# LMCache/LMCache

Hardware: AMD Instinct MI355X
Metric: KV encode+offload GB/s per GPU -- value = CacheGen encode, HBM -> HBM (raw 16-bit KV bytes consumed, PCIe never inside value); the PCIe-inclusive encode+offload rate is offload.encode_plus_offload_GBps_raw_kv (higher is better)
Workload: dtype bf16->u8 symbols (fp32 quantise, u32 rANS); 1 GPU; Llama-3-8B bf16 KV, 16384-token context, CacheGen encode, chunk_size=256 (BASELINE configs[1]); layers=32, kv_heads=8, head_dim=128, chunks=64, raw_kv_bytes=2147483648, numa_node=0

## Files before the change

lmcache_amd/csrc/k_encode_counts.h:

```cpp
#pragma once
#include "k_encode.h"

#define RTAB_ENTRIES 257
#define RTAB_DWORDS (2 * RTAB_ENTRIES + 2)
struct RansRtab {
  u32 v[RTAB_DWORDS];
};
constexpr RansRtab make_rans_rtab() {
  RansRtab t{};
  for (u32 c = 1; c <= 256u; c++) {
    const u32 f = 2u * c;
    u32 l = 1;
    while ((1u << l) < f) l++;
    const u64 num = 1ull << (31u + l);
    t.v[2 * c] = (u32)((num + f - 1u) / f);
    t.v[2 * c + 1] = (512u - f) | ((l - 1u) << 24);
  }
  return t;
}
__device__ const RansRtab g_rans_rtab = make_rans_rtab();
#define BITS_DWORDS 132
#define RTAB_LDS_DWORDS (RTAB_DWORDS + 2 * BITS_DWORDS)
struct CountsBits {
  u32 v[2 * BITS_DWORDS];
};
constexpr CountsBits make_counts_bits() {
  constexpr u16 t[257] = {LMC_COUNTS_BITS_LIST};
  constexpr u16 o[257] = {LMC_COUNTS_BPO_LIST};
  CountsBits r{};
  for (int i = 0; i < 257; i++) r.v[i >> 1] |= (u32)t[i] << (16 * (i & 1));
  for (int i = 0; i < 257; i++) r.v[BITS_DWORDS + (i >> 1)] |= (u32)o[i] << (16 * (i & 1));
  return r;
}
__device__ const CountsBits g_counts_bits = make_counts_bits();
#define CNT_RING_DWORDS 128

__device__ __forceinline__ void rtab_to_lds(u32* rtab_lds) {
  for (u32 i = threadIdx.x; i < RTAB_DWORDS; i += blockDim.x) rtab_lds[i] = g_rans_rtab.v[i];
  for (u32 i = threadIdx.x; i < 2 * BITS_DWORDS; i += blockDim.x) rtab_lds[RTAB_DWORDS + i] = g_counts_bits.v[i];
}

#define LMC_SYM_LAST_LOAD(p) __builtin_nontemporal_load((const LMC_GLOBAL u32*)(p))

#define CNT_TAB_DWORDS 1024

template <int POS, int WIDTH, int SHIFT>
__device__ __forceinline__ u32 row_addr_sh(u32 w, u32 base) {
  constexpr u32 FIELD = ((1u << WIDTH) - 1u);
  u32 r;
  if constexpr (POS == SHIFT) {
    asm("v_and_b32_e32 %0, %2, %1\n\tv_add_u32_e32 %0, %0, %3" : "=&v"(r) : "v"(w), "s"(FIELD << SHIFT), "v"(base));
  } else if constexpr (POS + WIDTH == 32) {
    asm("v_lshrrev_b32_e32 %0, %2, %1\n\tv_lshl_add_u32 %0, %0, %3, %4"
        : "=&v"(r) : "v"(w), "n"(POS), "n"(SHIFT), "v"(base));
  } else {
    asm("v_bfe_u32 %0, %1, %2, %3\n\tv_lshl_add_u32 %0, %0, %4, %5"
        : "=&v"(r) : "v"(w), "n"(POS), "n"(WIDTH), "n"(SHIFT), "v"(base));
  }
  return r;
}
template <bool NIB, int I, bool ALIGNED = false>
__device__ __forceinline__ u32 row_addr_cnt(const u32* w, u32 base) {
  if constexpr (NIB) {
    constexpr int POS = 8 * (I & 3) + 4 * ((I >> 2) & 1);
    if constexpr (ALIGNED && POS == 8) {
      u32 r;
      asm("v_and_or_b32 %0, %1, %2, %3" : "=v"(r) : "v"(w[I >> 3]), "s"(0xf00u), "v"(base));
      return r;
    } else if constexpr (ALIGNED && POS > 8) {
      u32 r;
      asm("v_lshrrev_b32_e32 %0, %2, %1\n\tv_and_or_b32 %0, %0, %3, %4" : "=&v"(r) : "v"(w[I >> 3]), "n"(POS - 8), "s"(0xf00u), "v"(base));
      return r;
    } else {
      return row_addr_sh<POS, 4, 8>(w[I >> 3], base);
    }
  } else {
    constexpr int POS = 8 * (I & 3);
    if constexpr (ALIGNED && POS >= 8) {
      u32 r;
      asm("v_lshrrev_b32_e32 %0, %2, %1\n\tv_and_or_b32 %0, %0, %3, %4" : "=&v"(r) : "v"(w[I >> 2]), "n"(POS - 7), "s"(0xf80u), "v"(base));
      return r;
    } else {
      return row_addr_sh<POS, 8, 7>(w[I >> 2], base);
    }
  }
}


struct CountsStream {
  int chunk, p, g, c;
  int T;
  bool active, nib;
  const u32* symq;
  u32 R;
};
__device__ __forceinline__ CountsStream counts_stream_of(const EncodeArgs& a, int chunk, int p, int g, int lane) {
  CountsStream s;
  s.g = g;
  s.p = p;
  s.chunk = chunk;
  s.c = s.g * 64 + lane;
  s.T = min(a.chunk_tokens, a.tok_end - (a.tok_begin + chunk * a.chunk_tokens));
  s.active = s.c < a.C;
  s.symq = a.sym4 + ((long long)s.chunk * a.P + s.p) * a.sym_stride + s.c;
  s.nib = lmc_sym_nibbles((int)a.bins.b[s.p]);
  s.R = (u32)a.bins.b[s.p] - 1u;
  return s;
}

struct CountsState {
  u32 pk[8];
  u32 wor[8];
  u32 head;
};

#define LMC_SDWA_BYTE_OP(NAME, OP)                                                                                      \
  template <int K>                                                                                                      \
  __device__ __forceinline__ u32 NAME(u32 a, u32 b) {                                                                   \
    u32 d;                                                                                                              \
    if constexpr (K == 0) asm(OP " %0, %1, %2 dst_sel:DWORD dst_unused:UNUSED_PAD src0_sel:DWORD src1_sel:BYTE_0" : "=v"(d) : "v"(a), "v"(b)); \
    else if constexpr (K == 1) asm(OP " %0, %1, %2 dst_sel:DWORD dst_unused:UNUSED_PAD src0_sel:DWORD src1_sel:BYTE_1" : "=v"(d) : "v"(a), "v"(b)); \
    else if constexpr (K == 2) asm(OP " %0, %1, %2 dst_sel:DWORD dst_unused:UNUSED_PAD src0_sel:DWORD src1_sel:BYTE_2" : "=v"(d) : "v"(a), "v"(b)); \
    else asm(OP " %0, %1, %2 dst_sel:DWORD dst_unused:UNUSED_PAD src0_sel:DWORD src1_sel:BYTE_3" : "=v"(d) : "v"(a), "v"(b)); \
    return d;                                                                                                           \
  }
LMC_SDWA_BYTE_OP(sdwa_byte_shl, "v_lshlrev_b32_sdwa")
LMC_SDWA_BYTE_OP(sdwa_byte_add, "v_add_u32_sdwa")
LMC_SDWA_BYTE_OP(sdwa_byte_or, "v_or_b32_sdwa")

template <int NS>
__device__ __forceinline__ void counts_model_pk(const u32 (&pk)[8], bool active, u32 T, u32 (&mp)[NS / 4]) {
  if (T == LMC_COUNTS_T) {
    u32 sum = 0;
#pragma unroll
    for (int k = 0; k < NS / 4; k++) sum = __builtin_amdgcn_sad_u8(pk[k], 0u, sum);
    const u32 deficit = LMC_COUNTS_T - sum;
    const bool first = (pk[0] & 0xffu) == 255u;
#pragma unroll
    for (int k = 0; k < NS / 4; k++) mp[k] = pk[k];
    mp[0] += first ? deficit << 8 : deficit;
  } else {
    const u32 magic = lmc_counts_scale_magic_dev(T);
    u32 cum = 0, prev = 0, big = 0, first = 0;
#pragma unroll
    for (int k = 0; k < NS / 4; k++) mp[k] = 0;
    static_for<NS>([&](auto itag) {
      constexpr int i = decltype(itag)::value;
      cum += (pk[i >> 2] >> (8 * (i & 3))) & 0xffu;
      const u32 now = __umulhi(cum << 8, magic);
      u32 n = now - prev;
      prev = now;
      if (n >= LMC_COUNTS_T) { big = 1u; first = i == 0 ? 1u : 0u; n = LMC_COUNTS_T - 1u; }
      mp[i >> 2] |= n << (8 * (i & 3));
    });
    if (big) mp[0] += first ? 1u << 8 : 1u;
  }
  if (!active) mp[0] = 0x01ffu;
}
__device__ __forceinline__ void counts_table_nib_pk(const u32 (&mp)[4], u32* tabmem, int lane) {
  u32 acc = 0;
  static_for<16>([&](auto itag) {
    constexpr int i = decltype(itag)::value;
    const u32 t = sdwa_byte_shl<i & 3>(23u, mp[i >> 2]);
    tabmem[i * 64 + lane] = (acc << 1) | t;
    acc = sdwa_byte_add<i & 3>(acc, mp[i >> 2]);
  });
}
__device__ __forceinline__ void counts_table_byte_pk(const u32 (&mp)[8], u16* tab16, int lane) {
  u32 acc = 0;
  static_for<32>([&](auto itag) {
    constexpr int i = decltype(itag)::value;
    tab16[i * 64 + lane] = (u16)sdwa_byte_or<i & 3>(acc << 8, mp[i >> 2]);
    acc = sdwa_byte_add<i & 3>(acc, mp[i >> 2]);
  });
}

template <bool ALIGNED = false, bool PLANE = false>
__device__ __forceinline__ u32 counts_hist_stream(const EncodeArgs& a, const CountsStream& s, u32* tabmem,
                                                  const u32* bits,
                                                  int lane, CountsState& cs, u32 vq_base = 0) {
  typedef __attribute__((address_space(3))) u32* lds_u32w;
  typedef const __attribute__((address_space(3))) u16* lds_u16p;
  typedef const __attribute__((address_space(3))) u8* lds_u8p;
  const int Tc = __builtin_amdgcn_readfirstlane(s.T);
  const u32 tab_addr = (u32)(size_t)(lds_u32w)tabmem;
  if (ALIGNED && (tab_addr & 0xfffu)) __builtin_trap();
  u16* const tab16 = reinterpret_cast<u16*>(tabmem);
  auto pass1 = [&](auto nib_tag) {
    constexpr bool NIB = decltype(nib_tag)::value;
    constexpr int DPB = NIB ? 4 : 8;
    const int NB = Tc >> 5, rem = Tc & 31;
    const int rows = NIB ? (Tc + 7) >> 3 : (Tc + 3) >> 2;
#pragma unroll
    for (int i = 0; i < 16; i++) tabmem[i * 64 + lane] = 0;
    const u32 col = NIB ? tab_addr + 4u * (u32)lane : tab_addr + 4u * (u32)(lane >> 1);
    const u32 one = NIB ? 1u : 1u << ((lane & 1) * 16);
    u32 w[DPB], wn[DPB];
#pragma unroll
    for (int j = 0; j < DPB; j++) w[j] = (s.active && j < rows) ? s.symq[(long long)j * a.C] : 0u;
    for (int b = 0; b < NB; b++) {
      if (b + 1 < NB || rem) {
#pragma unroll
        for (int j = 0; j < DPB; j++)
          wn[j] = (s.active && (b + 1) * DPB + j < rows) ? s.symq[(long long)((b + 1) * DPB + j) * a.C] : 0u;
      }
      static_for<32>([&](auto itag) {
        constexpr int i = decltype(itag)::value;
        const u32 ad = row_addr_cnt<NIB, i, ALIGNED>(w, col);
        __hip_atomic_fetch_add((lds_u32w)(size_t)ad, one, __ATOMIC_RELAXED, __HIP_MEMORY_SCOPE_WAVEFRONT);
      });
#pragma unroll
      for (int j = 0; j < DPB; j++) w[j] = wn[j];
    }
    for (int i = 0; i < rem; i++) {
      const int j = NIB ? i >> 3 : i >> 2;
      u32 wd = w[0];
#pragma unroll
      for (int k = 1; k < DPB; k++) wd = j == k ? w[k] : wd;
      const u32 sym = NIB ? (wd >> (8 * (i & 3) + 4 * ((i >> 2) & 1))) & 15u : (wd >> (8 * (i & 3))) & 0xffu;
      const u32 ad = col + (sym << (NIB ? 8 : 7));
      __hip_atomic_fetch_add((lds_u32w)(size_t)ad, one, __ATOMIC_RELAXED, __HIP_MEMORY_SCOPE_WAVEFRONT);
    }
  };
  const u32 vq = vq_base + (((u32)s.g) << 3) + ((u32)lane >> 3);
  const u32 qx = vq & 63u, qe = (u32)lane & 7u, qit = vq >> 6;
  u32 ph = 0;
  if constexpr (PLANE) {
    if (s.nib) {
      ph = (qit * 4u + (qe >> 1)) * 4096u + 4u * qx + 2u * (qe & 1u);
    } else {
      ph = (qit * 2u + (qe >> 2)) * 8192u + 4u * qx + (qe & 3u);
      const u32 sym0 = s.active ? (s.symq[0] & 0xffu) : 0u;
      const u32 a0 = ph + (sym0 << 8);
      const u32 c0 = (u32) * (lds_u8p)(size_t)a0;
      if (s.active && c0 != 255u)
        __hip_atomic_fetch_add((lds_u32w)(size_t)(a0 & ~3u), 1u << (8u * (a0 & 3u)), __ATOMIC_RELAXED, __HIP_MEMORY_SCOPE_WORKGROUP);
    }
  } else {
    if (s.nib) pass1(BoolTag<true>{});
    else pass1(BoolTag<false>{});
  }
  wave_lds_fence();

  if (s.g == 0) {
    const BlobOff bo = lmc_blob_off((u32)a.P, (u32)Tc, (u32)a.G);
    u8* const blob0 = a.blobs + (long long)s.chunk * a.blob_stride;
    const u32 sum = scale_checksum(reinterpret_cast<const u16*>(blob0 + bo.scales) + (long long)s.p * Tc, (u32)Tc, lane);
    if (lane == 0) reinterpret_cast<u32*>(blob0 + bo.scsum)[s.p] = sum;
  }
#pragma unroll
  for (int k = 0; k < 8; k++) cs.pk[k] = 0u;
  const u32 cap = s.active ? 255u : 0u;
  auto put = [&](auto itag, u32 c) {
    constexpr int i = decltype(itag)::value;
    if constexpr ((i & 3) == 0)
      asm("v_min_u32_sdwa %0, %1, %2 dst_sel:BYTE_0 dst_unused:UNUSED_PRESERVE src0_sel:DWORD src1_sel:DWORD" : "+v"(cs.pk[i >> 2]) : "v"(c), "v"(cap));
    else if constexpr ((i & 3) == 1)
      asm("v_min_u32_sdwa %0, %1, %2 dst_sel:BYTE_1 dst_unused:UNUSED_PRESERVE src0_sel:DWORD src1_sel:DWORD" : "+v"(cs.pk[i >> 2]) : "v"(c), "v"(cap));
    else if constexpr ((i & 3) == 2)
      asm("v_min_u32_sdwa %0, %1, %2 dst_sel:BYTE_2 dst_unused:UNUSED_PRESERVE src0_sel:DWORD src1_sel:DWORD" : "+v"(cs.pk[i >> 2]) : "v"(c), "v"(cap));
    else
      asm("v_min_u32_sdwa %0, %1, %2 dst_sel:BYTE_3 dst_unused:UNUSED_PRESERVE src0_sel:DWORD src1_sel:DWORD" : "+v"(cs.pk[i >> 2]) : "v"(c), "v"(cap));
  };
  if constexpr (PLANE) {
    if (s.nib) static_for<16>([&](auto itag) { put(itag, (u32) * (lds_u16p)(size_t)(ph + 256u * decltype(itag)::value)); });
    else static_for<32>([&](auto itag) { put(itag, (u32) * (lds_u8p)(size_t)(ph + 256u * decltype(itag)::value)); });
  } else {
    if (s.nib) static_for<16>([&](auto itag) { put(itag, tabmem[decltype(itag)::value * 64 + lane]); });
    else static_for<32>([&](auto itag) { put(itag, (u32)tab16[decltype(itag)::value * 64 + lane]); });
  }
  wave_lds_fence();
  head_or_counts<8>(cs.pk, cs.wor);
  cs.head = head_bytes_of<8, 8>(cs.wor, s.R);
  __builtin_assume(bits != nullptr);
  const u32 bits_addr = (u32)(size_t)(lds_u16p) reinterpret_cast<const u16*>(bits);
  u32 S = 0;
  auto bound = [&](auto ns_tag) {
    constexpr int NS = decltype(ns_tag)::value;
    u32 sum = 0;
#pragma unroll
    for (int k = 0; k < NS / 4; k++) sum = __builtin_amdgcn_sad_u8(cs.pk[k], 0u, sum);
    static_for<NS>([&](auto itag) {
      constexpr int i = decltype(itag)::value;
      u32 c2;
      if constexpr ((i & 3) == 0) asm("v_lshlrev_b32_sdwa %0, 1, %1 dst_sel:DWORD dst_unused:UNUSED_PAD src0_sel:DWORD src1_sel:BYTE_0" : "=v"(c2) : "v"(cs.pk[i >> 2]));
      else if constexpr ((i & 3) == 1) asm("v_lshlrev_b32_sdwa %0, 1, %1 dst_sel:DWORD dst_unused:UNUSED_PAD src0_sel:DWORD src1_sel:BYTE_1" : "=v"(c2) : "v"(cs.pk[i >> 2]));
      else if constexpr ((i & 3) == 2) asm("v_lshlrev_b32_sdwa %0, 1, %1 dst_sel:DWORD dst_unused:UNUSED_PAD src0_sel:DWORD src1_sel:BYTE_2" : "=v"(c2) : "v"(cs.pk[i >> 2]));
      else asm("v_lshlrev_b32_sdwa %0, 1, %1 dst_sel:DWORD dst_unused:UNUSED_PAD src0_sel:DWORD src1_sel:BYTE_3" : "=v"(c2) : "v"(cs.pk[i >> 2]));
      S += (u32) * (lds_u16p)(size_t)(c2 + bits_addr);
    });
    const u32 bits_of_1 = (u32) * (lds_u16p)(size_t)(bits_addr + 2u);
    S += sum == LMC_COUNTS_T - 1u ? bits_of_1 : 0u;
  };
  auto bound_T = [&](auto ns_tag) {
    constexpr int NS = decltype(ns_tag)::value;
    const u32 magic = lmc_counts_scale_magic_dev((u32)Tc);
    const u32 bpo_addr = bits_addr + 4u * BITS_DWORDS;
    u32 cum = 0, prev = 0;
    static_for<NS>([&](auto itag) {
      constexpr int i = decltype(itag)::value;
      const u32 c = (cs.pk[i >> 2] >> (8 * (i & 3))) & 0xffu;
      cum += c;
      const u32 now = __umulhi(cum << 8, magic);
      const u32 n = min(now - prev, LMC_COUNTS_T - 1u);
      prev = now;
      S += c * (u32) * (lds_u16p)(size_t)(bpo_addr + 2u * n);
    });
  };
  if (Tc == (int)LMC_COUNTS_T) {
    if (s.nib) bound(IntTag<16>{});
    else bound(IntTag<32>{});
  } else {
    if (s.nib) bound_T(IntTag<16>{});
    else bound_T(IntTag<32>{});
  }
  const u32 lw = s.active ? (S + 6u * ((S >> 12) + 2u)) >> 12 : 0u;
  const u32 words = (u32)__builtin_amdgcn_readfirstlane((int)wave_sum_u32(lw));
  return (cs.head + 2u * (words + 128u) + 15u) & ~15u;
}

__device__ __forceinline__ void counts_open_stream(const CountsStream& s, const CountsState& cs, u8* out, u32* tabmem, int lane) {
  (void)head_write<8, 8>(out, cs.pk, cs.wor, s.R, tabmem, lane);
  wave_lds_fence();
  if (s.nib) {
    u32 mp[4];
    counts_model_pk<16>(cs.pk, s.active, (u32)s.T, mp);
    counts_table_nib_pk(mp, tabmem, lane);
  } else {
    u32 mp[8];
    counts_model_pk<32>(cs.pk, s.active, (u32)s.T, mp);
    counts_table_byte_pk(mp, reinterpret_cast<u16*>(tabmem), lane);
  }
  wave_lds_fence();
}

template <bool NT>
__device__ __forceinline__ u32 counts_code_stream(const EncodeArgs& a, const CountsStream& s, u32* tabmem, u16* const ring,
                                                  const u32* rtab, int lane, u16* const out_v) {
  typedef __attribute__((address_space(3))) u32* lds_u32w;
  typedef __attribute__((address_space(3))) u16* lds_u16w;
  const int Tc = __builtin_amdgcn_readfirstlane(s.T);
  const u32 tab_addr = (u32)(size_t)(lds_u32w)tabmem;
  if (NT && (tab_addr & 0xfffu)) __builtin_trap();
  const u32 rtab_addr = (u32)__builtin_amdgcn_readfirstlane((int)(u32)(size_t)(lds_u32w) const_cast<u32*>(rtab));
  u32 x = s.active ? LMC_COUNTS_L : 0u;
  const u32 ring_addr = (u32)__builtin_amdgcn_readfirstlane((int)(u32)(size_t)(lds_u16w)ring);
  const u64 full_exec = __builtin_amdgcn_read_exec();
  u16* const out = reinterpret_cast<u16*>(uniform_ptr64(out_v));
  const u32 pre = (u32)__builtin_amdgcn_readfirstlane((int)((u32)(size_t)out & 255u));
  u32 skip = pre;
  u32 wb = ring_addr + pre;
  const u32 wlimit = ring_addr + 256u;
  u32 flushed = 0;
  const __amdgpu_buffer_rsrc_t out_rsrc = __builtin_amdgcn_make_buffer_rsrc((void*)((u8*)out - pre), (short)0, (int)0xfffffff0u, 0x00020000);
  auto flush_ring = [&]() {
    if (__builtin_expect(wb >= wlimit, 0)) {
      wave_lds_fence();
      u32 lane_here = (u32)lane;
      asm volatile("" : "+v"(lane_here));
      const u32 slot_addr = ring_addr + 4u * lane_here;
      const u32 v = *(lds_u32w)(size_t)slot_addr;
      const u32 up = *(lds_u32w)(size_t)(slot_addr + 256u);
      const u32 voff = 4u * lane_here;
#ifndef LMC_EXP_ENC_NO_FLUSH
      if (voff >= skip) __builtin_amdgcn_raw_buffer_store_b32((int)v, out_rsrc, (int)voff, (int)(flushed << 1), NT ? 2 : 0);
      skip = 0;
#else
      asm volatile("" :: "v"(v), "v"(voff));
#endif
      if (voff < wb - wlimit) *(lds_u32w)(size_t)slot_addr = up;
      flushed += 128u;
      wb -= 256u;
    }
  };
  auto rans_put_nib = [&](u32 e, u32 m, u32 shc) {
    u32 q;
    asm("v_mul_hi_u32 %[q], %[x], %[m]\n\t"
        "v_lshrrev_b32_sdwa %[q], %[shc], %[q] dst_sel:DWORD dst_unused:UNUSED_PAD src0_sel:BYTE_3 src1_sel:DWORD\n\t"
        "v_mad_u32_u24 %[x], %[q], %[shc], %[x]\n\t"
        "v_add_u32_sdwa %[x], %[x], %[e] dst_sel:DWORD dst_unused:UNUSED_PAD src0_sel:DWORD src1_sel:WORD_0"
        : [x] "+v"(x), [q] "=&v"(q)
        : [m] "v"(m), [shc] "v"(shc), [e] "v"(e));
  };
  auto rans_put_byte = [&](_Float16 e, u32 m, u32 shc) {
    u32 q, st2;
    asm("v_mul_hi_u32 %[q], %[x], %[m]\n\t"
        "v_lshrrev_b32_sdwa %[q], %[shc], %[q] dst_sel:DWORD dst_unused:UNUSED_PAD src0_sel:BYTE_3 src1_sel:DWORD\n\t"
        "v_lshlrev_b32_sdwa %[st2], 1, %[e] dst_sel:DWORD dst_unused:UNUSED_PAD src0_sel:DWORD src1_sel:BYTE_1\n\t"
        "v_mad_u32_u24 %[x], %[q], %[shc], %[x]\n\t"
        "v_add_u32_e32 %[x], %[x], %[st2]"
        : [x] "+v"(x), [q] "=&v"(q), [st2] "=&v"(st2)
        : [m] "v"(m), [shc] "v"(shc), [e] "v"(e));
  };

  auto pass2 = [&](auto nib_tag) {
    constexpr bool NIB = decltype(nib_tag)::value;
    constexpr int DPB = NIB ? 4 : 8;
    const int NB = Tc >> 5, rem = Tc & 31;
    const int rows = NIB ? (Tc + 7) >> 3 : (Tc + 3) >> 2;
    const u32 col = NIB ? tab_addr + 4u * (u32)lane : tab_addr + 2u * (u32)lane;
    using ET = std::conditional_t<NIB, u32, _Float16>;
    auto entry_at = [&](u32 ad) -> ET {
      if constexpr (NIB) return *(lds_u32w)(size_t)ad;
      else return __builtin_bit_cast(_Float16, *(lds_u16w)(size_t)ad);
    };
    auto rtab_of = [&](ET e) -> u32x2_t {
      u32 ra;
      if constexpr (NIB) ra = e >> 20;
      else ra = ((u32)__builtin_bit_cast(u16, e) & 0xffu) << 3;
      return *(const __attribute__((address_space(3))) u32x2_t*)(size_t)(rtab_addr + ra);
    };
    auto emit = [&](ET e0, ET e2, u32& ra) {
      u32 tt, cnt, wbn;
      if constexpr (NIB) {
        asm volatile("v_lshrrev_b32_e32 %[ra], 20, %[e2]\n\t"
                     "v_cmpx_ge_u32_sdwa vcc, %[x], %[e0] src0_sel:WORD_1 src1_sel:WORD_1\n\t"
                     "s_bcnt1_i32_b64 %[cnt], vcc\n\t"
                     "s_lshl1_add_u32 %[wbn], %[cnt], %[wb]\n\t"
                     "v_mbcnt_lo_u32_b32 %[t], vcc_lo, 0\n\t"
                     "v_mbcnt_hi_u32_b32 %[t], vcc_hi, %[t]\n\t"
                     "v_lshl_add_u32 %[t], %[t], 1, %[wb]\n\t"
                     "ds_write_b16 %[t], %[x]\n\t"
                     "v_lshrrev_b32_e32 %[x], 16, %[x]\n\t"
                     "s_mov_b64 exec, %[full]"
                     : [x] "+v"(x), [t] "=&v"(tt), [cnt] "=&s"(cnt), [wbn] "=&s"(wbn), [ra] "=&v"(ra)
                     : [e0] "v"(e0), [e2] "v"(e2), [wb] "s"(wb), [full] "s"(full_exec)
                     : "vcc", "scc", "memory");
      } else {
        asm volatile("v_lshlrev_b32_sdwa %[ra], 3, %[e2] dst_sel:DWORD dst_unused:UNUSED_PAD src0_sel:DWORD src1_sel:BYTE_0\n\t"
                     "v_lshlrev_b32_sdwa %[t], 23, %[e0] dst_sel:DWORD dst_unused:UNUSED_PAD src0_sel:DWORD src1_sel:BYTE_0\n\t"
                     "v_cmpx_ge_u32_e32 vcc, %[x], %[t]\n\t"
                     "s_bcnt1_i32_b64 %[cnt], vcc\n\t"
                     "s_lshl1_add_u32 %[wbn], %[cnt], %[wb]\n\t"
                     "v_mbcnt_lo_u32_b32 %[t], vcc_lo, 0\n\t"
                     "v_mbcnt_hi_u32_b32 %[t], vcc_hi, %[t]\n\t"
                     "v_lshl_add_u32 %[t], %[t], 1, %[wb]\n\t"
                     "ds_write_b16 %[t], %[x]\n\t"
                     "v_lshrrev_b32_e32 %[x], 16, %[x]\n\t"
                     "s_mov_b64 exec, %[full]"
                     : [x] "+v"(x), [t] "=&v"(tt), [cnt] "=&s"(cnt), [wbn] "=&s"(wbn), [ra] "=&v"(ra)
                     : [e0] "v"(e0), [e2] "v"(e2), [wb] "s"(wb), [full] "s"(full_exec)
                     : "vcc", "scc", "memory");
      }
      wb = wbn;
    };
    u32 w[DPB], wn[DPB];
#pragma unroll
    for (int j = 0; j < DPB; j++) {
      w[j] = (NB > 0 && s.active) ? LMC_SYM_LAST_LOAD(s.symq + (long long)((NB - 1) * DPB + j) * a.C) : 0u;
      wn[j] = (rem && s.active && NB * DPB + j < rows) ? LMC_SYM_LAST_LOAD(s.symq + (long long)(NB * DPB + j) * a.C) : 0u;
    }
    for (int i = rem - 1; i >= 0; i--) {
      const int j = NIB ? i >> 3 : i >> 2;
      u32 wd = wn[0];
#pragma unroll
      for (int k = 1; k < DPB; k++) wd = j == k ? wn[k] : wd;
      const u32 sym = NIB ? (wd >> (8 * (i & 3) + 4 * ((i >> 2) & 1))) & 15u : (wd >> (8 * (i & 3))) & 0xffu;
      const ET E = entry_at(col + (sym << (NIB ? 8 : 7)));
      const u32x2_t R = rtab_of(E);
      u32 ra_unused;
      emit(E, E, ra_unused);
      flush_ring();
      if constexpr (NIB) rans_put_nib(E, R.x, R.y);
      else rans_put_byte(E, R.x, R.y);
    }
#ifdef LMC_EXP_SKIP_TOKEN_LOOP
    return;
#endif
    if (NB == 0) return;
    ET E0 = entry_at(row_addr_cnt<NIB, 31, NT>(w, col));
    ET E1 = entry_at(row_addr_cnt<NIB, 30, NT>(w, col));
    ET E2 = entry_at(row_addr_cnt<NIB, 29, NT>(w, col));
    ET E3 = entry_at(row_addr_cnt<NIB, 28, NT>(w, col));
    u32x2_t R0 = rtab_of(E0);
    u32x2_t R1 = rtab_of(E1);
    for (int b = NB - 1; b >= 0; b--) {
#pragma unroll
      for (int j = 0; j < DPB; j++) wn[j] = (b > 0 && s.active) ? LMC_SYM_LAST_LOAD(s.symq + (long long)((b - 1) * DPB + j) * a.C) : 0u;
      static_for<32>([&](auto itag) {
        constexpr int i = 31 - decltype(itag)::value;
        u32 ad4;
        if constexpr (i >= 4) ad4 = row_addr_cnt<NIB, i - 4, NT>(w, col);
        else ad4 = row_addr_cnt<NIB, 28 + i, NT>(wn, col);
        u32 ra;
        emit(E0, E2, ra);
        const u32x2_t R2 = *(const __attribute__((address_space(3))) u32x2_t*)(size_t)(rtab_addr + ra);
        const ET E4 = entry_at(ad4);
        if constexpr ((i & 1) == 0) flush_ring();
        if constexpr (NIB) rans_put_nib(E0, R0.x, R0.y);
        else rans_put_byte(E0, R0.x, R0.y);
        E0 = E1; E1 = E2; E2 = E3; E3 = E4;
        R0 = R1; R1 = R2;
      });
#pragma unroll
      for (int j = 0; j < DPB; j++) w[j] = wn[j];
    }
  };
  if (s.nib) pass2(BoolTag<true>{});
  else pass2(BoolTag<false>{});
  x = s.active ? x : LMC_COUNTS_L;
  flush_ring();
  wave_lds_fence();
  const u32 pend_b = wb - ring_addr;
  {
    const u32 sa = wb + 4u * (u32)lane;
    *(lds_u16w)(size_t)sa = (u16)x;
    *(lds_u16w)(size_t)(sa + 2u) = (u16)(x >> 16);
  }
  wave_lds_fence();
  const u32 tot_b = pend_b + 256u;
  const u32 end_b = (tot_b + 15u) & ~15u;
  const u32 exact = (flushed << 1) + tot_b - pre;
#pragma unroll
  for (int h = 0; h < 2; h++) {
    const u32 voff = 256u * (u32)h + 4u * (u32)lane;
    if (voff < end_b && voff >= skip) {
      u32 v = *(lds_u32w)(size_t)(ring_addr + voff);
      v = voff >= tot_b ? 0u : (voff + 2u == tot_b ? (v & 0xffffu) : v);
      __builtin_amdgcn_raw_buffer_store_b32((int)v, out_rsrc, (int)voff, (int)(flushed << 1), NT ? 2 : 0);
    }
  }
  return exact;
}

template <bool QUADSYM, bool ENCODE, int NW = ENC_WAVES, bool COUNTS_ONLY = false>
__global__ __launch_bounds__(64 * NW) __attribute__((amdgpu_waves_per_eu(NW == 8 ? 8 : 4, 8))) void k_cdf_encode(EncodeArgs a) {
  static_assert(!COUNTS_ONLY || (QUADSYM && ENCODE), "the counts coder reads the workspace and places its streams");
  constexpr int TAB_DWORDS = COUNTS_ONLY ? CNT_TAB_DWORDS : ENC_TAB_DWORDS;
  constexpr int RING_DWORDS = COUNTS_ONLY ? CNT_RING_DWORDS : ENC_RING_DWORDS;
  __shared__ __attribute__((aligned(4096))) u32 lds_all[NW * (TAB_DWORDS + RING_DWORDS)];
  __shared__ __attribute__((aligned(16))) u32 rtab_lds[ENCODE ? RTAB_LDS_DWORDS : 4];
  if (ENCODE && QUADSYM) {
    rtab_to_lds(rtab_lds);
    __syncthreads();
  }
  const int lane = threadIdx.x & 63;
  const int wave = __builtin_amdgcn_readfirstlane((int)(threadIdx.x >> 6));
  const int npl = (COUNTS_ONLY && a.nplanes) ? a.nplanes : a.P;
  const long long ngroups_total = (long long)a.nchunks * npl * a.G;
  u32* hist = lds_all + wave * TAB_DWORDS;

  u32 item = blockIdx.x;
  if constexpr (ENCODE) item = (u32)__builtin_amdgcn_readfirstlane((int)draw_ticket(a.ticket, a.ticket_base));
  const u32 npg = (u32)(npl * a.G);
  u32 chunk_i, pg_i;
  if (ENCODE && npg % NW == 0) {
    chunk_i = item % (unsigned)a.nchunks;
    pg_i = (item / (unsigned)a.nchunks) * NW + (u32)wave;
  } else {
    const u32 lin = item * NW + (u32)wave;
    chunk_i = lin / npg;
    pg_i = lin - chunk_i * npg;
  }
  const long long gid = (long long)chunk_i * npg + pg_i;
  if (gid >= ngroups_total) return;
  PendingTile t;
  u16* const wring = reinterpret_cast<u16*>(lds_all + NW * TAB_DWORDS + wave * RING_DWORDS);
  u32 alloc = 0;
  auto counts_stream = [&]() {
    const u32 p_i = pg_i / (u32)a.G;
    const CountsStream s = counts_stream_of(a, (int)chunk_i, (int)p_i, (int)(pg_i - p_i * (u32)a.G), lane);
    CountsState cs;
    alloc = counts_hist_stream(a, s, hist, rtab_lds + RTAB_DWORDS, lane, cs);
    u8* const slot = a.scratch + gid * (long long)a.cap;
    counts_open_stream(s, cs, slot, hist, lane);
    t.exact = cs.head + counts_code_stream<false>(a, s, hist, wring, rtab_lds, lane, reinterpret_cast<u16*>(slot + cs.head));
    t.chunk = s.chunk; t.pg = s.p * a.G + s.g; t.T = (u32)s.T; t.out = reinterpret_cast<const u16*>(slot);
    if (lane == 0 && (t.exact > alloc || t.exact + 16 > a.cap)) atomicOr(a.status, LMC_ST_STREAM_OVERFLOW);
  };
  if constexpr (COUNTS_ONLY) {
    const int n = a.P * a.G;
    const u32 y_i = pg_i / (u32)a.G, g_i = pg_i - y_i * (u32)a.G;
    const int p_i = a.plane0 + (int)y_i * (a.plane_step ? a.plane_step : 1);
    CountsStream s = counts_stream_of(a, (int)chunk_i, p_i, (int)g_i, lane);
    s.symq = a.sym4 + ((long long)chunk_i * npl + y_i) * a.sym_stride + s.c;
    CountsState cs;
    alloc = counts_hist_stream<true>(a, s, hist, rtab_lds + RTAB_DWORDS, lane, cs);
    const bool layered = a.chain_gran != 0;
    const bool wave_gran = layered && (a.G % NW) != 0;
    const int kv = (layered && p_i >= a.L) ? 1 : 0;
    unsigned long long* const agg = layered ? a.agg + ((long long)chunk_i * 2 + kv) * a.L * a.chain_gran : a.agg + (long long)chunk_i * n;
    const int gi = layered ? (p_i - kv * a.L) * a.chain_gran + (int)(wave_gran ? g_i : g_i / NW) : (int)pg_i / NW;
    __shared__ u32 wg_alloc[NW];
    __shared__ u32 wg_excl;
    u32 beg, chain_end;
    if (!wave_gran) {
      if (lane == 0) wg_alloc[wave] = alloc;
      __syncthreads();
      u32 before = 0, wg_total = 0;
#pragma unroll
      for (int w = 0; w < NW; w++) {
        before += w < wave ? wg_alloc[w] : 0u;
        wg_total += wg_alloc[w];
      }
      if (wave == 0) {
        if (lane == 0 && gi > 0) agg_store(agg + gi, AGG_A, wg_total);
        const u32 e = lookback_exclusive(agg, gi, lane, a.status);
        if (lane == 0) {
          agg_store(agg + gi, AGG_P, e + wg_total);
          wg_excl = e;
        }
      }
      __syncthreads();
      beg = wg_excl + before;
      chain_end = wg_excl + wg_total;
    } else {
      if (lane == 0 && gi > 0) agg_store(agg + gi, AGG_A, alloc);
      beg = lookback_exclusive(agg, gi, lane, a.status);
      if (lane == 0) agg_store(agg + gi, AGG_P, beg + alloc);
      chain_end = beg + alloc;
    }
    const BlobOff bo = lmc_blob_off((u32)a.P, (u32)s.T, (u32)a.G);
    u8* const blob = a.blobs + (long long)chunk_i * a.blob_stride;
    u8* const out = kv ? a.vregion + (long long)chunk_i * a.vstride + beg : blob + bo.streams + beg;
    if (kv && (long long)beg + alloc > a.vstride) {
      if (lane == 0) atomicOr(a.status, LMC_ST_STREAM_OVERFLOW);
      return;
    }
    counts_open_stream(s, cs, out, hist, lane);
    const u32 exact = cs.head + counts_code_stream<true>(a, s, hist, wring, rtab_lds, lane, reinterpret_cast<u16*>(out + cs.head));
    const u32 padded = (exact + 15u) & ~15u;
    if (alloc > padded) zero_fill16(out + padded, alloc - padded, lane);
    if (lane == 0) {
      u32* d = reinterpret_cast<u32*>(blob + bo.gdir) + 2 * (p_i * a.G + (int)g_i);
      d[0] = beg;
      d[1] = beg + exact;
      if (exact > alloc) atomicOr(a.status, LMC_ST_STREAM_OVERFLOW);
    }
    if (!layered && (int)pg_i == n - 1) {
      write_blob_static(blob, bo, a, (u32)s.T, chain_end, lane);
      if (lane == 0) a.sizes[chunk_i] = bo.streams + chain_end;
    }
    return;
  } else if constexpr (ENCODE && QUADSYM) {
    const int chunk_of = (int)chunk_i;
    const bool counts_model =
        lmc_model_for_dev((u32)min(a.chunk_tokens, a.tok_end - (a.tok_begin + chunk_of * a.chunk_tokens))) == LMC_MODEL_COUNTS;
    if (counts_model) counts_stream();
    else {
      encode_group_stream<QUADSYM, ENCODE>(a, gid, hist, wring, lane, t);
      alloc = (t.exact + 15u) & ~15u;
    }
  } else {
    encode_group_stream<QUADSYM, ENCODE>(a, gid, hist, wring, lane, t);
    alloc = (t.exact + 15u) & ~15u;
  }
  if (!ENCODE) return;
  const int n = a.P * a.G;
  const int chunk = t.chunk;
  unsigned long long* agg = a.agg + (long long)chunk * n;
  if (n % NW == 0) {
    __shared__ u32 wg_alloc[NW];
    __shared__ u32 wg_excl;
    if (lane == 0) wg_alloc[wave] = alloc;
    __syncthreads();
    u32 before = 0, wg_total = 0;
#pragma unroll
    for (int w = 0; w < NW; w++) {
      before += w < wave ? wg_alloc[w] : 0u;
      wg_total += wg_alloc[w];
    }
    if (wave == 0) {
      const int wgi = t.pg / NW;
      if (lane == 0 && wgi > 0) agg_store(agg + wgi, AGG_A, wg_total);
      const u32 e = lookback_exclusive(agg, wgi, lane, a.status);
      if (lane == 0) {
        agg_store(agg + wgi, AGG_P, e + wg_total);
        wg_excl = e;
      }
    }
    __syncthreads();
    place_stream(a, t, wg_excl + before, alloc, wg_excl + wg_total, hist, lane);
  } else {
    if (lane == 0 && t.pg > 0) agg_store(agg + t.pg, AGG_A, alloc);
    const u32 excl = lookback_exclusive(agg, t.pg, lane, a.status);
    if (lane == 0) agg_store(agg + t.pg, AGG_P, excl + alloc);
    place_stream(a, t, excl, alloc, excl + alloc, hist, lane);
  }
}
```

lmcache_amd/csrc/k_fused.h:

```cpp
#pragma once
#include "k_encode_counts.h"
#include "k_quantize.h"

#define FUSED_MAX_NS 16
#define FUSED_WAVES 8
constexpr int FUSED_PRIO_A = 3;

#ifdef LMC_EXP_TIMELINE
__device__ unsigned long long g_fused_timeline[8192 * 8];
#define LMC_TL(k) do { if (threadIdx.x == 0 && tick < 8192u) g_fused_timeline[tick * 8u + (k)] = wall_clock64(); } while (0)
#else
#define LMC_TL(k) do { } while (0)
#endif
struct FusedArgs {
  KvAddr src;
  EncodeArgs e;
  u8* scale_base;
  long long scale_stride;
  u32 epoch;
  int pl, ipc;
  u32 item_base;
};

template <bool PSRC>
__device__ __forceinline__ long long fused_tok_off(const KvAddr& a, int t) {
  if constexpr (!PSRC) return lmc_tok_off(a, t);
  else {
    const unsigned long long ad = uniform_ptr64(a.slot_mapping + t);
    const u32 s = *(const __attribute__((address_space(4))) u32*)ad;
    const u32 bs = (u32)a.block_size;
    const u32 b = s >> (u32)__builtin_ctz(bs), w = s & (bs - 1u);
    return (long long)b * a.stride_block + (long long)w * a.stride_token;
  }
}

template <int NITER, int DT, bool NIB, bool FULL, bool ALLROWS, bool PSRC = false>
__device__ __forceinline__ void quantize_oct(const KvAddr& src, const typename KvElem<DT>::T* pbase, int tok0, int Tc, int t_first,
                                             bool q1valid, bool skip0, int C, float maxf, u32* sym_out, u16* scale_out,
                                             int lane) {
  long long coff[NITER];
  int c0[NITER];
  bool cval[NITER];
#pragma unroll
  for (int it = 0; it < NITER; it++) {
    c0[it] = (it * 64 + lane) * 8;
    cval[it] = FULL || c0[it] < C;
    const int h = c0[it] / src.D, d = c0[it] - h * src.D;
    coff[it] = (long long)h * src.stride_head + d;
  }
  const f32x2_t maxf2 = {maxf, maxf};
  const u32 lane4 = 4u * (u32)lane;
  u32 o[NITER][8];
  u32 ad[2] = {lane4, lane4};
  auto hist_dword = [&](auto it_tag, auto e_tag, auto hq_tag, u32 od) {
    constexpr int it = decltype(it_tag)::value, e = decltype(e_tag)::value, hq = decltype(hq_tag)::value;
    plane_hist_dword<NIB, it, e, hq>(od, ad, [&](int row) { return (ALLROWS || t_first + row < Tc) && (NIB || !(row == 0 && skip0)); });
  };
#pragma unroll
  for (int q = 0; q < 4; q++) {
    const int rowi[2] = {NIB ? q : 2 * q, NIB ? q + 4 : 2 * q + 1};
    uint4 v[2][NITER];
    bool tv[2];
#pragma unroll
    for (int r = 0; r < 2; r++) {
      const int t = t_first + rowi[r];
      tv[r] = ALLROWS || t < Tc;
      const typename KvElem<DT>::T* rowp = pbase + (tv[r] ? fused_tok_off<PSRC>(src, tok0 + t) : 0);
#pragma unroll
      for (int it = 0; it < NITER; it++) {
        if (tv[r] && (FULL || cval[it])) v[r][it] = kv_ld8<DT, true>(rowp + coff[it]);
        else v[r][it] = make_uint4(0, 0, 0, 0);
      }
    }
    u32 mrow[2];
#pragma unroll
    for (int r = 0; r < 2; r++) {
      u32 m = 0;
#pragma unroll
      for (int it = 0; it < NITER; it++) {
        m = kv_absmax8<DT>(m, v[r][it]);
      }
      mrow[r] = max(m & 0xffffu, m >> 16);
    }
    wave_max2_u32(mrow[0], mrow[1]);
    mrow[0] = kv_max_scale<DT>(mrow[0]);
    mrow[1] = kv_max_scale<DT>(mrow[1]);
    if (lane == 0) {
#pragma unroll
      for (int r = 0; r < 2; r++)
        if (tv[r]) scale_out[rowi[r]] = (u16)mrow[r];
    }
    float factor[2];
    bool special[2] = {false, false};
    u32 slow = 0;
    const bool short_div = row_div_in_range(mrow[0], lmc_math_dtype(DT)) && row_div_in_range(mrow[1], lmc_math_dtype(DT));
    if (short_div) {
#pragma unroll
      for (int r = 0; r < 2; r++) factor[r] = row_div_short(maxf, h2f_rt(mrow[r], lmc_math_dtype(DT)));
    } else {
      bool any_special = false;
#pragma unroll
      for (int r = 0; r < 2; r++) {
        const float sf = h2f_rt(mrow[r], lmc_math_dtype(DT));
        factor[r] = maxf / sf;
        special[r] = !(__builtin_fabsf(factor[r]) < __builtin_inff()) || !(sf < __builtin_inff());
        any_special |= special[r];
      }
      slow = __ballot(any_special) != 0 ? 1u : 0u;
    }
#pragma unroll
    for (int it = 0; it < NITER; it++) {
      if (!FULL && !cval[it]) continue;
#pragma unroll
      for (int r = 0; r < 2; r++) {
        const u32 w[4] = {v[r][it].x, v[r][it].y, v[r][it].z, v[r][it].w};
        const int bpos = NIB ? q : (2 * q + r) & 3;
        const bool fresh = NIB ? (q == 0 && r == 0) : bpos == 0;
        const bool high = NIB && r == 1;
        if (slow == 0u) {
          const f32x2_t f2 = {factor[r], factor[r]};
#pragma unroll
          for (int k = 0; k < 4; k++) {
            const f32x2_t z = quant_z2(kv_lo<DT>(w, k), kv_hi<DT>(w, k), f2, maxf2);
            if (high) {
              asm("v_lshl_or_b32 %0, %1, %2, %0" : "+v"(o[it][2 * k]) : "v"(__builtin_amdgcn_cvt_pk_u8_f32(z.x, 0, 0u)), "n"(8 * bpos + 4));
              asm("v_lshl_or_b32 %0, %1, %2, %0" : "+v"(o[it][2 * k + 1]) : "v"(__builtin_amdgcn_cvt_pk_u8_f32(z.y, 0, 0u)), "n"(8 * bpos + 4));
            } else {
              o[it][2 * k] = __builtin_amdgcn_cvt_pk_u8_f32(z.x, bpos, fresh ? 0u : o[it][2 * k]);
              o[it][2 * k + 1] = __builtin_amdgcn_cvt_pk_u8_f32(z.y, bpos, fresh ? 0u : o[it][2 * k + 1]);
            }
          }
        } else {
#pragma unroll
          for (int k = 0; k < 4; k++) {
            const float xl = kv_lo<DT>(w, k), xh = kv_hi<DT>(w, k);
            const u32 sl_ = (special[r] ? quant_special(xl, factor[r], maxf) : quant_fast(xl, factor[r], maxf)) & 0xffu;
            const u32 sh_ = (special[r] ? quant_special(xh, factor[r], maxf) : quant_fast(xh, factor[r], maxf)) & 0xffu;
            o[it][2 * k] = (fresh ? 0u : o[it][2 * k]) | sl_ << (8 * bpos + (high ? 4 : 0));
            o[it][2 * k + 1] = (fresh ? 0u : o[it][2 * k + 1]) | sh_ << (8 * bpos + (high ? 4 : 0));
          }
        }
      }
    }
    if (NIB ? q == 3 : (q & 1) == 1) {
      const int hq = NIB ? 0 : q >> 1;
#pragma unroll
      for (int it = 0; it < NITER; it++) {
        if (!FULL && !cval[it]) continue;
        if (!NIB && hq == 1 && !q1valid) continue;
        u32* dst = sym_out + (NIB ? 0ll : (long long)hq * C) + c0[it];
        *reinterpret_cast<uint4*>(dst) = make_uint4(o[it][0], o[it][1], o[it][2], o[it][3]);
        *reinterpret_cast<uint4*>(dst + 4) = make_uint4(o[it][4], o[it][5], o[it][6], o[it][7]);
      }
#ifndef LMC_EXP_SKIP_HIST
      static_for<NITER>([&](auto it_tag) {
        constexpr int it = decltype(it_tag)::value;
        if (FULL || cval[it]) {
          static_for<8>([&](auto e_tag) {
            constexpr int e = decltype(e_tag)::value;
            if (q < 2) hist_dword(it_tag, e_tag, IntTag<0>{}, o[it][e]);
            else hist_dword(it_tag, e_tag, IntTag<1>{}, o[it][e]);
          });
        }
      });
#endif
    }
  }
}

template <int GL, int NITER, int DT, int NW, bool PSRC = false>
__global__ __launch_bounds__(64 * NW) __attribute__((amdgpu_waves_per_eu(8, 8))) void k_encode_fused(FusedArgs fa) {
  static_assert(GL == 64 || NITER == 1, "narrow planes: one channel run per lane");
  const EncodeArgs& a = fa.e;
  static_assert(NW * CNT_TAB_DWORDS == PLANE_HIST_DWORDS, "the workgroup's table slices are the plane's histogram");
  constexpr bool HISTA = GL == 64;
  constexpr bool HISTN = GL == 32;
  __shared__ __attribute__((aligned(HISTA ? 32768 : 4096))) u32 lds_all[NW * (CNT_TAB_DWORDS + CNT_RING_DWORDS)];
  __shared__ __attribute__((aligned(16))) u32 rtab_lds[RTAB_LDS_DWORDS];
  __shared__ u32 st_alloc[FUSED_MAX_NS];
  __shared__ u32 wg_excl;
  __shared__ u32 wg_ticket;
  const int lane = threadIdx.x & 63;
  const int wave = __builtin_amdgcn_readfirstlane((int)(threadIdx.x >> 6));
#ifdef LMC_EXP_TIMELINE
  const unsigned long long tl_pre = wall_clock64();
#endif
  typedef __attribute__((address_space(3))) u32* lds_u32w;
  constexpr bool EARLY = GL != 32;
  u32 tick;
  if constexpr (EARLY) {
    u32 tk = 0;
    if (threadIdx.x == 0) tk = __hip_atomic_fetch_add(a.ticket, 1u, __ATOMIC_RELAXED, __HIP_MEMORY_SCOPE_AGENT);
    if constexpr (HISTA) {
      if ((u32)(size_t)(lds_u32w)lds_all != 0u) __builtin_trap();
      uint4* z = reinterpret_cast<uint4*>(lds_all);
#pragma unroll
      for (int i = 0; i < PLANE_HIST_DWORDS / 4 / (64 * NW); i++) z[i * 64 * NW + threadIdx.x] = make_uint4(0, 0, 0, 0);
    }
    rtab_to_lds(rtab_lds);
    if (threadIdx.x == 0) wg_ticket = tk - a.ticket_base;
    __syncthreads();
    tick = (u32)__builtin_amdgcn_readfirstlane((int)wg_ticket);
  } else {
    tick = (u32)__builtin_amdgcn_readfirstlane((int)draw_ticket(a.ticket, a.ticket_base));
  }
  const u32 item = fa.item_base + tick;
  LMC_TL(0);
#ifdef LMC_EXP_TIMELINE
  if (threadIdx.x == 0 && tick < 8192u) {
    u32 hwid, xcc;
    asm volatile("s_getreg_b32 %0, hwreg(HW_REG_HW_ID)" : "=s"(hwid));
    asm volatile("s_getreg_b32 %0, hwreg(HW_REG_XCC_ID)" : "=s"(xcc));
    g_fused_timeline[tick * 8u + 6u] = ((unsigned long long)xcc << 32) | hwid;
    g_fused_timeline[tick * 8u + 7u] = tl_pre;
  }
#endif
  const int chunk = (int)(item % (unsigned)a.nchunks), it = (int)(item / (unsigned)a.nchunks);
  const int p0 = it * fa.pl, np = min(fa.pl, a.P - p0);
  const int NS = np * a.G;
  const int tok0 = a.tok_begin + chunk * a.chunk_tokens;
  const int Tc = a.chunk_tokens;
  u32* const hist = lds_all + wave * CNT_TAB_DWORDS;
  u16* const ring = reinterpret_cast<u16*>(lds_all + NW * CNT_TAB_DWORDS + wave * CNT_RING_DWORDS);

  if constexpr (!EARLY) rtab_to_lds(rtab_lds);
  const bool hist_a = HISTA || (HISTN && np * GL <= 128);
  if constexpr (!EARLY) {
    if ((u32)(size_t)(lds_u32w)lds_all != 0u) __builtin_trap();
    if (hist_a) {
      uint4* z = reinterpret_cast<uint4*>(lds_all);
#pragma unroll
      for (int i = 0; i < PLANE_HIST_DWORDS / 4 / (64 * NW); i++) z[i * 64 * NW + threadIdx.x] = make_uint4(0, 0, 0, 0);
      __syncthreads();
    }
  }
  if (p0 + np == a.P && threadIdx.x == 64 * (NW - 1)) a.sizes[chunk] = 0u;
  {
    const int TO = (Tc + 7) >> 3;
    u8* const scl0 = fa.scale_base + (long long)chunk * fa.scale_stride;
    __builtin_amdgcn_s_setprio(FUSED_PRIO_A);
    if constexpr (GL < 64) {
      constexpr int RPW = 64 / GL;
      const int OG = (TO + RPW - 1) / RPW;
      const int sub = lane / GL, sl = lane % GL;
#pragma unroll 1
      for (int task = wave; task < np * OG; task += NW) {
        const int p = p0 + task / OG;
        int oct = (task % OG) * RPW + sub;
        const bool ovalid = oct < TO;
        if (!ovalid) oct = 0;
        const int bins = (int)a.bins.b[p];
        const float maxf = (float)(bins / 2 - 1);
        const bool nib = lmc_sym_nibbles(bins);
        u32* const sym_out = const_cast<u32*>(a.sym4) + ((long long)chunk * a.P + p) * a.sym_stride + (long long)oct * (nib ? 1 : 2) * a.C;
        u16* const scale_out = reinterpret_cast<u16*>(scl0) + (long long)p * Tc + oct * 8;
        const bool q1valid = 2 * oct + 1 < a.TQ;
        if (HISTN && hist_a) {
          const u32 vq = (u32)((task / OG) * GL + sl);
          const u32 hl4 = 4u * (vq & 63u);
          const int hit = __builtin_amdgcn_readfirstlane((int)(((u32)(task / OG) * GL) >> 6));
          if (nib) quantize_task<GL, 1, DT, true, true, 4, 2, 1, true>(fa.src, p, tok0, Tc, oct * 8, ovalid, q1valid, a.C, maxf, sym_out, nullptr, scale_out, sl, 0, nullptr, hl4, hit);
          else quantize_task<GL, 1, DT, true, false, 4, 2, 1, true>(fa.src, p, tok0, Tc, oct * 8, ovalid, q1valid, a.C, maxf, sym_out, nullptr, scale_out, sl, 0, nullptr, hl4, hit);
        } else if (nib) quantize_task<GL, 1, DT, true, true, 4, 2>(fa.src, p, tok0, Tc, oct * 8, ovalid, q1valid, a.C, maxf, sym_out, nullptr, scale_out, sl);
        else quantize_task<GL, 1, DT, true, false, 4, 2>(fa.src, p, tok0, Tc, oct * 8, ovalid, q1valid, a.C, maxf, sym_out, nullptr, scale_out, sl);
      }
    } else {
      const int p = p0;
      const int bins = (int)a.bins.b[p];
      const float maxf = (float)(bins / 2 - 1);
      const bool nib = lmc_sym_nibbles(bins);
      const bool full = a.C == NITER * 512;
      u32* const sym_pc = const_cast<u32*>(a.sym4) + ((long long)chunk * a.P + p) * a.sym_stride;
      u16* const scl = reinterpret_cast<u16*>(scl0) + (long long)p * Tc;
      const typename KvElem<DT>::T* const pbase = lmc_plane_base<typename KvElem<DT>::T>(fa.src, p);
#ifdef LMC_EXP_SKIP_PHASE_A
      if (false)
#endif
#pragma unroll 1
      for (int oct = wave; oct < TO; oct += NW) {
        const bool q1valid = 2 * oct + 1 < a.TQ;
        const bool allrows = oct * 8 + 8 <= Tc;
        u32* const so = sym_pc + (long long)oct * (nib ? 1 : 2) * a.C;
        if (!allrows) {
          if (nib) quantize_oct<NITER, DT, true, false, false, PSRC>(fa.src, pbase, tok0, Tc, oct * 8, q1valid, oct == 0, a.C, maxf, so, scl + oct * 8, lane);
          else quantize_oct<NITER, DT, false, false, false, PSRC>(fa.src, pbase, tok0, Tc, oct * 8, q1valid, oct == 0, a.C, maxf, so, scl + oct * 8, lane);
        } else if (full) {
          if (nib) quantize_oct<NITER, DT, true, true, true, PSRC>(fa.src, pbase, tok0, Tc, oct * 8, q1valid, oct == 0, a.C, maxf, so, scl + oct * 8, lane);
          else quantize_oct<NITER, DT, false, true, true, PSRC>(fa.src, pbase, tok0, Tc, oct * 8, q1valid, oct == 0, a.C, maxf, so, scl + oct * 8, lane);
        } else if (nib) quantize_oct<NITER, DT, true, false, true, PSRC>(fa.src, pbase, tok0, Tc, oct * 8, q1valid, oct == 0, a.C, maxf, so, scl + oct * 8, lane);
        else quantize_oct<NITER, DT, false, false, true, PSRC>(fa.src, pbase, tok0, Tc, oct * 8, q1valid, oct == 0, a.C, maxf, so, scl + oct * 8, lane);
      }
    }
    __builtin_amdgcn_s_setprio(0);
  }
  __syncthreads();
  LMC_TL(1);

  auto stream_of = [&](int j) -> CountsStream {
    const int pj = (int)((u32)j / (u32)a.G);
    return counts_stream_of(a, chunk, p0 + pj, j - pj * a.G, lane);
  };
  CountsState cs0, cs1;
  auto pass1 = [&](int j, CountsState& cs) {
    if (j < NS) {
      const CountsStream s = stream_of(j);
      u32 alloc;
      if (HISTA) alloc = counts_hist_stream<true, true>(a, s, hist, rtab_lds + RTAB_DWORDS, lane, cs);
      else if (HISTN && hist_a) alloc = counts_hist_stream<true, true>(a, s, hist, rtab_lds + RTAB_DWORDS, lane, cs, (u32)(s.p - p0) * GL);
      else alloc = counts_hist_stream<true>(a, s, hist, rtab_lds + RTAB_DWORDS, lane, cs);
      if (lane == 0) st_alloc[j] = alloc;
    }
  };
  pass1(wave, cs0);
  pass1(wave + NW, cs1);
  __syncthreads();
  LMC_TL(2);

  u32 wg_total = 0;
  for (int j = 0; j < NS; j++) wg_total += st_alloc[j];
  if (wave == 0) {
    unsigned long long* agg = a.agg + (long long)chunk * fa.ipc;
    if (lane == 0 && it > 0) agg_store(agg + it, AGG_A, wg_total, fa.epoch);
    const u32 e = lookback_exclusive<true>(agg, it, lane, a.status, fa.epoch);
    if (lane == 0) {
      agg_store(agg + it, AGG_P, e + wg_total, fa.epoch);
      wg_excl = e;
    }
  }
  __syncthreads();
  LMC_TL(3);

  const BlobOff bo = lmc_blob_off((u32)a.P, (u32)Tc, (u32)a.G);
  u8* const blob = a.blobs + (long long)chunk * a.blob_stride;
  auto pass2 = [&](int j, const CountsState& cs) {
    if (j < NS) {
      u32 beg = wg_excl;
      for (int k = 0; k < j; k++) beg += st_alloc[k];
      const u32 alloc = st_alloc[j];
      const CountsStream s = stream_of(j);
      u8* const out = blob + bo.streams + beg;
      counts_open_stream(s, cs, out, hist, lane);
      const u32 exact = cs.head + counts_code_stream<true>(a, s, hist, ring, rtab_lds, lane, reinterpret_cast<u16*>(out + cs.head));
      const u32 padded = (exact + 15u) & ~15u;
      if (alloc > padded) zero_fill16(out + padded, alloc - padded, lane);
      if (lane == 0) {
        u32* d = reinterpret_cast<u32*>(blob + bo.gdir) + 2 * (s.p * a.G + s.g);
        d[0] = beg;
        d[1] = beg + exact;
        if (exact > alloc) atomicOr(a.status, LMC_ST_STREAM_OVERFLOW);
      }
      wave_lds_fence();
    }
  };
  pass2(wave, cs0);
  pass2(wave + NW, cs1);
#ifdef LMC_EXP_TIMELINE
  LMC_TL(4);
  __syncthreads();
  LMC_TL(5);
#endif
  if (p0 + np == a.P && wave == NW - 1) {
    write_blob_static<lmc_dtype_fp8(DT) ? DT : 0>(blob, bo, a, (u32)Tc, wg_excl + wg_total, lane);
    if (lane == 0) a.sizes[chunk] = bo.streams + wg_excl + wg_total;
  }
}
```

Baseline: 2721 GB/s.

## Load symbol rows via buffer descriptors with scalar offsets and reorder rANS scheduling

Symbol word loads in both counting and coding passes now use raw buffer loads with a per-stream resource descriptor. A scalar offset walks the rows, and out-of-bounds rows or inactive lanes return zero through the hardware range check, replacing per-load 64-bit address math and predicates. The rANS put asm blocks become volatile with memory clobbers, a sched_barrier is inserted, and the next LDS entry lookup moves after the put. These pin the instruction order in the hot loop. The blob offset is also made wave-uniform via readfirstlane, which cuts VGPR and address cost but risks scheduling regressions from the tighter ordering constraints.

Measured after the change: 2753 GB/s, median of 6. +1.1%, better.

```diff
diff --git a/lmcache_amd/csrc/k_encode_counts.h b/lmcache_amd/csrc/k_encode_counts.h
--- a/lmcache_amd/csrc/k_encode_counts.h
+++ b/lmcache_amd/csrc/k_encode_counts.h
@@ -40,7 +40,7 @@
   for (u32 i = threadIdx.x; i < 2 * BITS_DWORDS; i += blockDim.x) rtab_lds[RTAB_DWORDS + i] = g_counts_bits.v[i];
 }
 
-#define LMC_SYM_LAST_LOAD(p) __builtin_nontemporal_load((const LMC_GLOBAL u32*)(p))
+#define LMC_SYM_LAST_LOAD(rsrc, voff, soff) ((u32)__builtin_amdgcn_raw_buffer_load_b32(rsrc, (int)(voff), (int)(soff), 2 ))
 
 #define CNT_TAB_DWORDS 1024
 
@@ -108,6 +108,25 @@
   return s;
 }
 
+struct SymBlocks {
+  __amdgpu_buffer_rsrc_t rsrc;
+  u32 voff;
+  u32 rowb;
+  __device__ __forceinline__ u32 load(u32 soff) const { return (u32)__builtin_amdgcn_raw_buffer_load_b32(rsrc, (int)voff, (int)soff, 0); }
+  __device__ __forceinline__ u32 load_last(u32 soff) const { return LMC_SYM_LAST_LOAD(rsrc, voff, soff); }
+  __device__ __forceinline__ u32 load_tail(u32 row) const { return (u32)__builtin_amdgcn_raw_buffer_load_b32(rsrc, (int)(voff + row * rowb), 0, 0); }
+  __device__ __forceinline__ u32 load_tail_last(u32 row) const { return LMC_SYM_LAST_LOAD(rsrc, voff + row * rowb, 0); }
+};
+__device__ __forceinline__ SymBlocks sym_blocks_of(const EncodeArgs& a, const CountsStream& s, int rows) {
+  SymBlocks sb;
+  u32 rowb = (u32)__builtin_amdgcn_readfirstlane(4 * a.C);
+  asm volatile("" : "+s"(rowb));
+  sb.rowb = rowb;
+  sb.voff = s.active ? 4u * (u32)s.c : 0x40000000u;
+  sb.rsrc = __builtin_amdgcn_make_buffer_rsrc((void*)uniform_ptr64(s.symq - s.c), (short)0, (int)((u32)rows * rowb), 0x00020000);
+  return sb;
+}
+
 struct CountsState {
   u32 pk[8];
   u32 wor[8];
@@ -195,14 +214,23 @@
     for (int i = 0; i < 16; i++) tabmem[i * 64 + lane] = 0;
     const u32 col = NIB ? tab_addr + 4u * (u32)lane : tab_addr + 4u * (u32)(lane >> 1);
     const u32 one = NIB ? 1u : 1u << ((lane & 1) * 16);
+    const SymBlocks sb = sym_blocks_of(a, s, rows);
     u32 w[DPB], wn[DPB];
 #pragma unroll
-    for (int j = 0; j < DPB; j++) w[j] = (s.active && j < rows) ? s.symq[(long long)j * a.C] : 0u;
+    for (int j = 0; j < DPB; j++) w[j] = sb.load_tail((u32)j);
+    u32 soff = 0;
     for (int b = 0; b < NB; b++) {
-      if (b + 1 < NB || rem) {
-#pragma unroll
-        for (int j = 0; j < DPB; j++)
-          wn[j] = (s.active && (b + 1) * DPB + j < rows) ? s.symq[(long long)((b + 1) * DPB + j) * a.C] : 0u;
+      soff += (u32)DPB * sb.rowb;
+      if (b + 1 < NB) {
+        u32 so = soff;
+#pragma unroll
+        for (int j = 0; j < DPB; j++) {
+          wn[j] = sb.load(so);
+          so += sb.rowb;
+        }
+      } else if (rem) {
+#pragma unroll
+        for (int j = 0; j < DPB; j++) wn[j] = sb.load_tail((u32)((b + 1) * DPB + j));
       }
       static_for<32>([&](auto itag) {
         constexpr int i = decltype(itag)::value;
@@ -375,22 +403,24 @@
   };
   auto rans_put_nib = [&](u32 e, u32 m, u32 shc) {
     u32 q;
-    asm("v_mul_hi_u32 %[q], %[x], %[m]\n\t"
+    asm volatile("v_mul_hi_u32 %[q], %[x], %[m]\n\t"
         "v_lshrrev_b32_sdwa %[q], %[shc], %[q] dst_sel:DWORD dst_unused:UNUSED_PAD src0_sel:BYTE_3 src1_sel:DWORD\n\t"
         "v_mad_u32_u24 %[x], %[q], %[shc], %[x]\n\t"
         "v_add_u32_sdwa %[x], %[x], %[e] dst_sel:DWORD dst_unused:UNUSED_PAD src0_sel:DWORD src1_sel:WORD_0"
         : [x] "+v"(x), [q] "=&v"(q)
-        : [m] "v"(m), [shc] "v"(shc), [e] "v"(e));
+        : [m] "v"(m), [shc] "v"(shc), [e] "v"(e)
+        : "memory");
   };
   auto rans_put_byte = [&](_Float16 e, u32 m, u32 shc) {
     u32 q, st2;
-    asm("v_mul_hi_u32 %[q], %[x], %[m]\n\t"
+    asm volatile("v_mul_hi_u32 %[q], %[x], %[m]\n\t"
         "v_lshrrev_b32_sdwa %[q], %[shc], %[q] dst_sel:DWORD dst_unused:UNUSED_PAD src0_sel:BYTE_3 src1_sel:DWORD\n\t"
         "v_lshlrev_b32_sdwa %[st2], 1, %[e] dst_sel:DWORD dst_unused:UNUSED_PAD src0_sel:DWORD src1_sel:BYTE_1\n\t"
         "v_mad_u32_u24 %[x], %[q], %[shc], %[x]\n\t"
         "v_add_u32_e32 %[x], %[x], %[st2]"
         : [x] "+v"(x), [q] "=&v"(q), [st2] "=&v"(st2)
-        : [m] "v"(m), [shc] "v"(shc), [e] "v"(e));
+        : [m] "v"(m), [shc] "v"(shc), [e] "v"(e)
+        : "memory");
   };
 
   auto pass2 = [&](auto nib_tag) {
@@ -444,11 +474,23 @@
       }
       wb = wbn;
     };
+    const SymBlocks sb = sym_blocks_of(a, s, rows);
+    const u32 blockb = (u32)DPB * sb.rowb;
+    u32 soff = (u32)max(NB - 1, 0) * blockb;
     u32 w[DPB], wn[DPB];
 #pragma unroll
-    for (int j = 0; j < DPB; j++) {
-      w[j] = (NB > 0 && s.active) ? LMC_SYM_LAST_LOAD(s.symq + (long long)((NB - 1) * DPB + j) * a.C) : 0u;
-      wn[j] = (rem && s.active && NB * DPB + j < rows) ? LMC_SYM_LAST_LOAD(s.symq + (long long)(NB * DPB + j) * a.C) : 0u;
+    for (int j = 0; j < DPB; j++) w[j] = wn[j] = 0u;
+    if (NB > 0) {
+      u32 so = soff;
+#pragma unroll
+      for (int j = 0; j < DPB; j++) {
+        w[j] = sb.load_last(so);
+        so += sb.rowb;
+      }
+    }
+    if (rem) {
+#pragma unroll
+      for (int j = 0; j < DPB; j++) wn[j] = sb.load_tail_last((u32)(NB * DPB + j));
     }
     for (int i = rem - 1; i >= 0; i--) {
       const int j = NIB ? i >> 3 : i >> 2;
@@ -464,6 +506,8 @@
       if constexpr (NIB) rans_put_nib(E, R.x, R.y);
       else rans_put_byte(E, R.x, R.y);
     }
+#pragma unroll
+    for (int j = 0; j < DPB; j++) wn[j] = 0u;
 #ifdef LMC_EXP_SKIP_TOKEN_LOOP
     return;
 #endif
@@ -472,11 +516,19 @@
     ET E1 = entry_at(row_addr_cnt<NIB, 30, NT>(w, col));
     ET E2 = entry_at(row_addr_cnt<NIB, 29, NT>(w, col));
     ET E3 = entry_at(row_addr_cnt<NIB, 28, NT>(w, col));
+    __builtin_amdgcn_sched_barrier(0);
     u32x2_t R0 = rtab_of(E0);
     u32x2_t R1 = rtab_of(E1);
     for (int b = NB - 1; b >= 0; b--) {
-#pragma unroll
-      for (int j = 0; j < DPB; j++) wn[j] = (b > 0 && s.active) ? LMC_SYM_LAST_LOAD(s.symq + (long long)((b - 1) * DPB + j) * a.C) : 0u;
+      if (b > 0) {
+        soff -= blockb;
+        u32 so = soff;
+#pragma unroll
+        for (int j = 0; j < DPB; j++) {
+          wn[j] = sb.load_last(so);
+          so += sb.rowb;
+        }
+      }
       static_for<32>([&](auto itag) {
         constexpr int i = 31 - decltype(itag)::value;
         u32 ad4;
@@ -485,10 +537,10 @@
         u32 ra;
         emit(E0, E2, ra);
         const u32x2_t R2 = *(const __attribute__((address_space(3))) u32x2_t*)(size_t)(rtab_addr + ra);
-        const ET E4 = entry_at(ad4);
         if constexpr ((i & 1) == 0) flush_ring();
         if constexpr (NIB) rans_put_nib(E0, R0.x, R0.y);
         else rans_put_byte(E0, R0.x, R0.y);
+        const ET E4 = entry_at(ad4);
         E0 = E1; E1 = E2; E2 = E3; E3 = E4;
         R0 = R1; R1 = R2;
       });
diff --git a/lmcache_amd/csrc/k_fused.h b/lmcache_amd/csrc/k_fused.h
--- a/lmcache_amd/csrc/k_fused.h
+++ b/lmcache_amd/csrc/k_fused.h
@@ -336,6 +336,7 @@
     if (j < NS) {
       u32 beg = wg_excl;
       for (int k = 0; k < j; k++) beg += st_alloc[k];
+      beg = (u32)__builtin_amdgcn_readfirstlane((int)beg);
       const u32 alloc = st_alloc[j];
       const CountsStream s = stream_of(j);
       u8* const out = blob + bo.streams + beg;
```
